# andimarafioti/faster-qwen3-tts

Hardware: AMD Instinct MI355X
Metric: real-time factor (audio s / wall s), Qwen3-TTS-12Hz-0.6B voice-clone streaming chunk_size=8; p50 TTFA in ttfa_ms_p50 (higher is better)
Workload: dtype bf16

## Files before the change

### faster-qwen3-tts_amd/csrc/fq3_api.hip

```cpp
#define FQ3_SKINNY_EXTERN
#include "fq3_ctx.h"
#include "sampler.cuh"
#include "sampler_wave.cuh"
#include "skinny_gemm.cuh"
#include "state_kernels.cuh"

#include <cstdio>
#include <cstdlib>
#include <cstring>
#include <map>
#include <string>
#include <type_traits>
#include <vector>

using namespace fq3;

static thread_local std::string g_err;
static int fail(int code, const std::string& m) { g_err = m; return code; }
int fq3_fail_(int code, const std::string& m) { return fail(code, m); }
#define HIPCHK(x) do { hipError_t e_ = (x); if (e_ != hipSuccess) return fail(FQ3_EHIP, std::string(#x) + ": " + hipGetErrorString(e_)); } while (0)

extern "C" const char* fq3_last_error(void) { return g_err.c_str(); }
extern "C" void fq3_set_error_(const char* msg) { g_err = msg ? msg : ""; }
extern "C" int fq3_abi_version(void) { return FQ3_ABI_VERSION; }
// ... 196 lines not shown
    if ((r = dmalloc(c, &c->past_hidden, (size_t)t.hidden * c->esz))) return r;
    if ((r = dmalloc(c, &c->ph_hold, (size_t)t.hidden * c->esz))) return r;
    if ((r = dmalloc(c, &c->pred_in, (size_t)2 * t.hidden * c->esz))) return r;
    if ((r = dmalloc(c, &c->pred_next, (size_t)t.hidden * c->esz))) return r;
    if ((r = dmalloc(c, &c->pred_x, (size_t)p.hidden * c->esz))) return r;
    if ((r = dmalloc(c, &c->plogits, (size_t)(G - 1) * p.vocab * c->esz))) return r;
    const int maxkv = std::max(t.n_kv_heads, p.n_kv_heads);
    c->part_stride = (size_t)maxkv * kMaxWorkers * 4 * kPartStride;
    if ((r = dmalloc(c, (void**)&c->part, 2 * c->part_stride * sizeof(float)))) return r;
    if ((r = dmalloc(c, (void**)&c->rope_now, 2 * 64 * sizeof(float)))) return r;
    if ((r = dmalloc(c, (void**)&c->seen_api, kMaxVocab))) return r;
    if ((r = dmalloc(c, (void**)&c->st, sizeof(DecodeState)))) return r;
    if ((r = dmalloc(c, (void**)&c->seen, kMaxVocab))) return r;
    if ((r = dmalloc(c, (void**)&c->codes, (size_t)(frames + 1) * G * sizeof(int)))) return r;
    if ((r = dmalloc(c, (void**)&c->ids64, (size_t)64 * sizeof(int64_t)))) return r;
    if ((r = dmalloc(c, (void**)&c->d_pemb, (size_t)64 * sizeof(void*)))) return r;
    HIPCHK(hipStreamCreateWithFlags(&c->cap_stream, hipStreamNonBlocking));
    return FQ3_OK;
}

extern "C" int fq3_set_option(fq3_ctx* c, const char* key, int value) {
    if (!c || !key) return fail(FQ3_EINVAL, "null argument");
    const std::string k(key);
    if (k == "weight_nt") c->opt_nt = value;
    else if (k == "pred_m2") c->opt_m2 = value;
    else if (k == "pred_attn") c->opt_pred_attn = value;
    else if (k == "rows_per_wave_max") c->opt_rmax = value;
    else if (k == "prefill_mode") c->prefill_mode = value;
    else if (k == "flash_prefill") c->opt_flash_prefill = value;
    else if (k == "flash_small") c->opt_flash_small = value;
    else if (k == "cont_pack") c->opt_cont_pack = value;
    else if (k == "swiglu_tile") c->opt_swiglu_tile = value;
    else if (k == "packed_weights") c->opt_packed = value;
    else if (k == "skinny_gemm") c->opt_no_skinny = !value;
    else return fail(FQ3_EINVAL, "unknown option: " + k);
    fq3_graph_reset(c);
    return FQ3_OK;
}

extern "C" int fq3_graph_reset(fq3_ctx* c) {
    if (!c) return fail(FQ3_EINVAL, "null ctx");
    if (c->exec) { (void)hipGraphExecDestroy(c->exec); c->exec = nullptr; }
    if (c->graph) { (void)hipGraphDestroy(c->graph); c->graph = nullptr; }
    return FQ3_OK;
}

namespace {
struct PackedEntry { void* p; int refs; int N, K; };
std::mutex g_packed_mu;
std::map<std::pair<const void*, int>, PackedEntry> g_packed;
}
const void* fq3_packed_find_(const void* W, int kind) {
    std::lock_guard<std::mutex> lk(g_packed_mu);
    auto it = g_packed.find({W, kind});
    return it == g_packed.end() ? nullptr : it->second.p;
}
int fq3_packed_acquire_(const void* W, int N, int K, int kind) {
    if (!W || !skinny_pack_ok(N, K) || (kind == 1 && (N / 2) % 8) || (kind == 2 && N % 512)) return FQ3_EUNSUPPORTED;
    std::lock_guard<std::mutex> lk(g_packed_mu);
    auto it = g_packed.find({W, kind});
    if (it != g_packed.end()) {
        if (it->second.N != N || it->second.K != K) return fail(FQ3_EINVAL, "a matrix is bound with two different shapes");
        ++it->second.refs;
        return FQ3_OK;
    }
    void* p = nullptr;
    if (hipMalloc(&p, (size_t)N * K * 2) != hipSuccess) { (void)hipGetLastError(); return fail(FQ3_ENOMEM, "no device memory for the fragment-major weight copy"); }
    skinny_pack(reinterpret_cast<const bf16_t*>(W), reinterpret_cast<bf16_t*>(p), N, K, kind == 1 ? N / 2 : (kind == 2 ? -(N / 2) : 0), nullptr);
    if (hipStreamSynchronize(nullptr) != hipSuccess) { (void)hipFree(p); return fail(FQ3_EHIP, "packing a weight matrix failed"); }
    g_packed[{W, kind}] = PackedEntry{p, 1, N, K};
    return FQ3_OK;
}
void fq3_packed_release_(const void* W, int kind) {
    std::lock_guard<std::mutex> lk(g_packed_mu);
    auto it = g_packed.find({W, kind});
    if (it == g_packed.end()) return;
    if (--it->second.refs <= 0) { (void)hipFree(it->second.p); g_packed.erase(it); }
}
static void packed_release_all(fq3_ctx* c) {
    for (auto& r : c->packed_refs) fq3_packed_release_(r.first, r.second);
    c->packed_refs.clear();
}
static int packed_acquire_all(fq3_ctx* c) {
    if (c->cfg.dtype != FQ3_BF16) return FQ3_OK;
    auto take = [&](const void* W, int N, int K, int kind) -> int {
        const int r = fq3_packed_acquire_(W, N, K, kind);
        if (r == FQ3_OK) c->packed_refs.emplace_back(W, kind);
        return r == FQ3_EUNSUPPORTED ? FQ3_OK : r;
    };
    auto stack = [&](const std::vector<fq3_layer_weights>& L, const fq3_stack_dims& d) -> int {
        const int qd = d.n_heads * kHeadDim, kvd = d.n_kv_heads * kHeadDim;
        for (const fq3_layer_weights& l : L) {
            if (int r = take(l.qkv, qd + 2 * kvd, d.hidden, 0)) return r;
            if (int r = take(l.o, d.hidden, qd, 0)) return r;
            if (int r = take(l.gate_up, 2 * d.inter, d.hidden, 1)) return r;
            if (int r = take(l.gate_up, 2 * d.inter, d.hidden, 0)) return r;
            if (int r = take(l.down, d.hidden, d.inter, 0)) return r;
        }
        return FQ3_OK;
    };
    if (int r = stack(c->tl, c->cfg.talker)) return r;
    if (int r = stack(c->pl, c->cfg.predictor)) return r;
    for (const fq3_layer_weights& l : c->tl) if (int r = take(l.gate_up, 2 * c->cfg.talker.inter, c->cfg.talker.hidden, 2)) return r;
    if (int r = take(c->wt.codec_head, c->cfg.talker.vocab, c->cfg.talker.hidden, 0)) return r;
    for (const void* h : c->lmh) if (int r = take(h, c->cfg.predictor.vocab, c->cfg.predictor.hidden, 0)) return r;
    return FQ3_OK;
}

extern "C" int fq3_ctx_destroy(fq3_ctx* c) {
    if (!c) return FQ3_OK;
    (void)hipDeviceSynchronize();
    fq3_graph_reset(c);
    packed_release_all(c);
    if (c->cap_stream) (void)hipStreamDestroy(c->cap_stream);
    if (fq3_kv_pool* p = c->tk.pool) {
        (void)fq3_kv_release(c, 0);
        bool last;
        { std::lock_guard<std::mutex> lk(p->mu); last = --p->users == 0; }
        if (p->is_private && last) pool_free_(p);
    }
    for (void* p : c->allocs) (void)hipFree(p);
    delete c;
    return FQ3_OK;
}

extern "C" int fq3_bind_weights(fq3_ctx* c, const fq3_weight_table* w) {
    if (!c || !w) return fail(FQ3_EINVAL, "null argument");
    const int G = c->cfg.num_code_groups;
    if (!w->talker_layers || !w->predictor_layers || !w->codec_embedding || !w->codec_head || !w->talker_final_norm ||
        !w->predictor_final_norm || !w->predictor_embeddings || !w->lm_heads || !w->talker_cos || !w->talker_sin ||
        !w->pred_cos || !w->pred_sin)
        return fail(FQ3_EINVAL, "weight table has null entries");
    if (c->cfg.has_projection && !w->proj_w) return fail(FQ3_EINVAL, "has_projection set but proj_w is null");
    if (w->talker_rope_len < c->cfg.max_seq_len || w->pred_rope_len < G + 1)
        return fail(FQ3_EINVAL, "rope tables shorter than the caches");
    c->wt = *w;
    c->tl.assign(w->talker_layers, w->talker_layers + c->cfg.talker.n_layers);
    c->pl.assign(w->predictor_layers, w->predictor_layers + c->cfg.predictor.n_layers);
    c->pemb.assign(w->predictor_embeddings, w->predictor_embeddings + (G - 1));
    c->lmh.assign(w->lm_heads, w->lm_heads + (G - 1));
    for (auto& l : c->tl) if (!l.qkv || !l.o || !l.gate_up || !l.down || !l.input_norm || !l.post_norm || !l.q_norm || !l.k_norm)
        return fail(FQ3_EINVAL, "talker layer has null weights");
    for (auto& l : c->pl) if (!l.qkv || !l.o || !l.gate_up || !l.down || !l.input_norm || !l.post_norm || !l.q_norm || !l.k_norm)
        return fail(FQ3_EINVAL, "predictor layer has null weights");
    HIPCHK(hipMemcpy(c->d_pemb, c->pemb.data(), (G - 1) * sizeof(void*), hipMemcpyHostToDevice));
    (void)hipDeviceSynchronize();
    packed_release_all(c);
    if (int r = packed_acquire_all(c)) { packed_release_all(c); return r; }
    c->bound = true;
    fq3_graph_reset(c);
    return FQ3_OK;
}

template <typename T, int NCH, int PRO, int EPI, bool NT, int M = 1>
static void launch_gemv_n(const GemvArgs& a, int rmax, hipStream_t s) {
    const int R = gemv_rows_per_wave<NCH, EPI>(a.N, rmax);
    const int grid = gemv_grid(a.N, R);
    const size_t shm = gemv_lds_bytes<PRO, M>(a.K);
    if constexpr (MaxRows<NCH, EPI>::v >= 2) {
        if (R == 2) { gemv_launch<T, NCH, PRO, EPI, NT, M, 2>(a, grid, shm, s); return; }
    }
    gemv_launch<T, NCH, PRO, EPI, NT, M, 1>(a, grid, shm, s);
}
template <typename T, int PRO, int EPI>
static int launch_gemv2_t(const GemvArgs& a, int rmax, hipStream_t s) {
    constexpr int most = gemv_most_chunks(PRO, 2);
    const int n = gemv_chunks(a.K, most);
    if (!n) return fail(FQ3_EUNSUPPORTED, PRO == PRO_NORM ? "code predictor hidden size above 2048" : "code predictor GEMV inner dimension above 3072");
    with_value<1, 2, 4, 6>(n, [&](auto nch) {
        if constexpr (decltype(nch)::value <= most) launch_gemv_n<T, decltype(nch)::value, PRO, EPI, false, 2>(a, rmax, s);
    });
    return 0;
}
template <int PRO, int EPI>
static int launch_gemv2(const fq3_ctx* c, const GemvArgs& a, hipStream_t s) {
    return c->cfg.dtype == FQ3_BF16 ? launch_gemv2_t<bf16_t, PRO, EPI>(a, c->opt_rmax, s) : launch_gemv2_t<float, PRO, EPI>(a, c->opt_rmax, s);
}
template <typename T, int PRO, int EPI, bool NT>
static int launch_gemv_t(const GemvArgs& a, int rmax, hipStream_t s) {
    constexpr int most = gemv_most_chunks(PRO, 1);
    const int n = gemv_chunks(a.K, most);
    if (!n) return fail(FQ3_EUNSUPPORTED, PRO == PRO_NORM ? "hidden size above 2048" : "GEMV inner dimension above 6144");
    with_value<1, 2, 4, 6, 12>(n, [&](auto nch) {
        if constexpr (decltype(nch)::value <= most) launch_gemv_n<T, decltype(nch)::value, PRO, EPI, NT>(a, rmax, s);
    });
    return 0;
}
template <int PRO, int EPI>
static int launch_gemv(const fq3_ctx* c, const GemvArgs& a, bool nt, hipStream_t s) {
    const int rmax = c->opt_rmax;
    if (c->cfg.dtype == FQ3_BF16)
        return nt ? launch_gemv_t<bf16_t, PRO, EPI, true>(a, rmax, s) : launch_gemv_t<bf16_t, PRO, EPI, false>(a, rmax, s);
    return nt ? launch_gemv_t<float, PRO, EPI, true>(a, rmax, s) : launch_gemv_t<float, PRO, EPI, false>(a, rmax, s);
}

template <typename T, bool PAGED>
static void launch_attn_p(const AttnArgs& a, int rep, int workers, hipStream_t s) {
    with_value<1, 2, 4>(rep, [&](auto r) {
        attn_decode_launch<T, decltype(r)::value, PAGED>(a, workers, s);
    });
}
template <typename T>
static void launch_attn_t(const AttnArgs& a, int rep, int workers, hipStream_t s) {
    if (a.table) launch_attn_p<T, true>(a, rep, workers, s); else launch_attn_p<T, false>(a, rep, workers, s);
}

struct StepSrc { const void* x0; const int* pos_ptr; int pos_imm; bool kv_only_tail = false; };

static int run_stack(fq3_ctx* c, bool talker, const StepSrc& src, hipStream_t s) {
    const fq3_stack_dims& d = talker ? c->cfg.talker : c->cfg.predictor;
    const std::vector<fq3_layer_weights>& L = talker ? c->tl : c->pl;
    StackBufs& kv = talker ? c->tk : c->pk;
    const int rep = d.n_heads / d.n_kv_heads;
    const int q_dim = d.n_heads * kHeadDim, kv_dim = d.n_kv_heads * kHeadDim;
    const bool nt = c->opt_nt == 2 || (c->opt_nt == 1 && talker);
    const float *cos_row, *sin_row;
    if (src.pos_ptr) { cos_row = c->rope_now; sin_row = c->rope_now + 64; }
    else {
        const int rl = talker ? c->wt.talker_rope_len : c->wt.pred_rope_len;
        int rp = src.pos_imm + (talker ? c->rope_delta : 0);
        rp = rp < 0 ? 0 : (rp >= rl ? rl - 1 : rp);
        cos_row = (talker ? c->wt.talker_cos : c->wt.pred_cos) + (size_t)rp * 64;
        sin_row = (talker ? c->wt.talker_sin : c->wt.pred_sin) + (size_t)rp * 64;
    }
    for (int i = 0; i < d.n_layers; ++i) {
        const fq3_layer_weights& w = L[i];
        const void* xin = i == 0 ? src.x0 : c->h;
        GemvArgs g{};
        g.eps = d.rms_eps;
        g.W = w.qkv; g.N = q_dim + 2 * kv_dim; g.K = d.hidden; g.x = xin;
        g.norm_w = w.input_norm; g.y = c->qkv;
        if (int r = launch_gemv<PRO_NORM, EPI_STORE>(c, g, nt, s)) return r;
        const bool tail_skip = src.kv_only_tail && i == d.n_layers - 1;
        GemvArgs o{};
        o.W = w.o; o.N = d.hidden; o.K = q_dim; o.y = c->h; o.res = xin; o.rep = rep;
        AttnArgs a{};
        a.qkv = c->qkv; a.q_norm_w = w.q_norm; a.k_norm_w = w.k_norm; a.eps = d.rms_eps;
        a.cos_row = cos_row; a.sin_row = sin_row;
        a.kcache = kv.k[i]; a.vcache = kv.v[i]; a.max_seq = kv.max_seq;
        a.table = kv.d_table; a.blk_stride = kv.pool ? (int)kv.pool->blk_elems : 0;
        a.pos_ptr = src.pos_ptr; a.pos_imm = src.pos_imm;
        a.done_ptr = src.pos_ptr ? &c->st->done : nullptr;
        a.n_pad = talker ? c->n_pad : 0;
        a.n_kv = d.n_kv_heads; a.part = c->part;
        a.scale = 1.0f / sqrtf((float)kHeadDim);
        a.rep = rep; a.out = c->attn_out;
        const bool pred_attn = c->opt_pred_attn && !talker && !src.pos_ptr && src.pos_imm <= 16;
        if (pred_attn) {
            if (c->cfg.dtype == FQ3_BF16) attn_pred_launch<bf16_t>(a, d.n_heads, s);
            else attn_pred_launch<float>(a, d.n_heads, s);
            if (tail_skip) break;
            o.x = c->attn_out;
            if (int r = launch_gemv<PRO_PLAIN, EPI_RESIDUAL>(c, o, nt, s)) return r;
        } else {
            if (c->cfg.dtype == FQ3_BF16) launch_attn_t<bf16_t>(a, rep, kv.workers, s);
            else launch_attn_t<float>(a, rep, kv.workers, s);
            if (tail_skip) break;
            o.part = c->part; o.n_part = kv.workers;
            if (int r = launch_gemv<PRO_COMBINE, EPI_RESIDUAL>(c, o, nt, s)) return r;
        }
        GemvArgs m{};
        m.eps = d.rms_eps; m.W = w.gate_up; m.N = d.inter; m.K = d.hidden; m.x = c->h;
        m.norm_w = w.post_norm; m.y = c->act; m.up_off = d.inter;
        if (int r = launch_gemv<PRO_NORM, EPI_SWIGLU>(c, m, nt, s)) return r;
        GemvArgs dn{};
// ... 364 lines not shown
                g_err = m;
                return r;
            }
    }
    if (walk) {
        for (int q = 0; q < n; ++q)
            if (int r = fq3_prefill_continue(ctxs[q], embeds[q], start[q], cnt[q], out_logits ? out_logits[q] : nullptr, out_hidden[q], stream)) return r;
        return FQ3_OK;
    }
    for (int q = 0; q < n; ++q)
        if (int r = fq3_set_generation_state(ctxs[q], 0, 0)) return r;
    if (int r = fq3_prefill_continue_batch_mfma_(ctxs, n, embeds, start, cnt, out_logits, out_hidden, s)) return r;
    LAUNCH_CHECK();
    return FQ3_OK;
}

int fq3_codec_head_launch_(fq3_ctx* c, const void* hidden, void* out_logits, hipStream_t s) {
    GemvArgs g{};
    g.W = c->wt.codec_head; g.N = c->cfg.talker.vocab; g.K = c->cfg.talker.hidden; g.x = hidden; g.y = out_logits;
    return launch_gemv<PRO_PLAIN, EPI_STORE>(c, g, true, s);
}

extern "C" int fq3_set_prefill_mode(fq3_ctx* c, int mode) { return fq3_set_option(c, "prefill_mode", mode); }

__global__ void build_seen_kernel(const int64_t* history, int n, unsigned char* seen, int V) {
    for (int i = threadIdx.x; i < V; i += blockDim.x) seen[i] = 0;
    __syncthreads();
    for (int i = threadIdx.x; i < n; i += blockDim.x) { const int id = (int)history[i]; if (id >= 0 && id < V) seen[id] = 1; }
}

template <typename T>
static void launch_sample_pred(const DecodeState* st, const T* lg, int V, int cb, const SampleCfg& cfg, const T* nz,
                               int* codes, int G, int64_t* out64, const T* next_emb, T* next_in, int H, bool wave,
                               const TeacherForcing* tf, hipStream_t s) {
    if (wave) dispatch_nc(V, [&](auto nc) {
        constexpr int NC = decltype(nc)::value;
        sample_pred_wave_launch<T, NC>(st, lg, V, cb, cfg, nz, codes, G, out64, next_emb, next_in, H, tf, s);
    });
    else hipLaunchKernelGGL((sample_pred_kernel<T>), dim3(1), dim3(256), 0, s, st, lg, V, cb, cfg, nz, codes, G, out64,
                            next_emb, next_in, H, tf);
}
template <typename T>
static void launch_sample_talker(DecodeState* st, const T* lg, int V, const unsigned char* seen, int G, bool wave,
                                 const TeacherForcing* tf, hipStream_t s) {
    if (wave) dispatch_nc(V, [&](auto nc) {
        constexpr int NC = decltype(nc)::value;
        sample_talker_wave_launch<T, NC>(st, lg, V, seen, G, tf, s);
    });
    else hipLaunchKernelGGL((sample_talker_kernel<T>), dim3(1), dim3(256), 0, s, st, lg, V, seen, G, tf);
}
template <typename T>
static void launch_sample_api(fq3_ctx* c, const T* lg, int V, const SampleCfg& cfg, const int64_t* history, int n_hist,
                              const T* noise, int64_t* out, hipStream_t s) {
    if (cfg.top_p >= 1.0f) {
        const unsigned char* seen = nullptr;
        if (n_hist > 0) {
            hipLaunchKernelGGL(build_seen_kernel, dim3(1), dim3(256), 0, s, history, n_hist, c->seen_api, V);
            seen = c->seen_api;
        }
        dispatch_nc(V, [&](auto nc) {
            constexpr int NC = decltype(nc)::value;
            hipLaunchKernelGGL((sample_api_wave_kernel<T, NC>), dim3(1), dim3(256), 0, s, lg, V, cfg, seen, noise, out);
        });
    } else {
        hipLaunchKernelGGL((sample_api_kernel<T>), dim3(1), dim3(256), 0, s, lg, V, cfg, history, n_hist, noise, out);
    }
}

static SampleCfg to_cfg(const fq3_sampling& s) {
    SampleCfg c{};
// ... 20 lines not shown
    LAUNCH_CHECK();
    return FQ3_OK;
}

template <typename T>
__global__ __launch_bounds__(256) void rep_penalty_kernel(T* logits, int V, const unsigned char* seen, float penalty) {
    for (int i = threadIdx.x; i < V; i += 256) {
        if (!seen[i]) continue;
        const float v = DT<T>::ld(logits + i);
        DT<T>::st(logits + i, v > 0.f ? v / penalty : v * penalty);
    }
}
extern "C" int fq3_apply_repetition_penalty(fq3_ctx* c, void* logits, int V, const int64_t* history, int n_hist,
                                            float penalty, void* stream) {
    if (!c || !logits) return fail(FQ3_EINVAL, "null argument");
    if (V <= 0 || V > kMaxVocab) return fail(FQ3_EUNSUPPORTED, "vocab must be at most 4096");
    if (penalty == 1.0f || n_hist <= 0 || !history) return FQ3_OK;
    hipStream_t s = (hipStream_t)stream;
    hipLaunchKernelGGL(build_seen_kernel, dim3(1), dim3(256), 0, s, history, n_hist, c->seen_api, V);
    if (c->cfg.dtype == FQ3_BF16) hipLaunchKernelGGL((rep_penalty_kernel<bf16_t>), dim3(1), dim3(256), 0, s, (bf16_t*)logits, V, c->seen_api, penalty);
    else hipLaunchKernelGGL((rep_penalty_kernel<float>), dim3(1), dim3(256), 0, s, (float*)logits, V, c->seen_api, penalty);
    LAUNCH_CHECK();
    return FQ3_OK;
}

extern "C" int fq3_set_predictor_sampling(fq3_ctx* c, const fq3_sampling* s) {
    if (!c || !s) return fail(FQ3_EINVAL, "null argument");
    if (s->do_sample && !(s->temperature > 0.f)) return fail(FQ3_EINVAL, "temperature must be > 0");
    if ((s->top_p >= 1.0f) != (c->pred_sampling.top_p >= 1.0f)) fq3_graph_reset(c);
    c->pred_sampling = *s;
    return FQ3_OK;
}

template <typename T>
static int predictor_passes_t(fq3_ctx* c, const DecodeState* st_dev, const void* pred_input, const void* noise_imm,
                              int64_t* out64, void* out_logits, hipStream_t s) {
    const fq3_stack_dims &p = c->cfg.predictor, &t = c->cfg.talker;
    const int G = c->cfg.num_code_groups, Vp = p.vocab, Ht = t.hidden;
    SampleCfg scfg = to_cfg(c->pred_sampling);
    for (int pass = 0; pass < G; ++pass) {
        const void* hsrc = c->h;
        if (pass == 0 && c->opt_m2) {
            const T* xa = (const T*)pred_input;
            const T* xb = (const T*)pred_input + Ht;
            if (c->cfg.has_projection) {
                GemvArgs g{};
                g.W = c->wt.proj_w; g.bias = c->wt.proj_b; g.N = p.hidden; g.K = Ht; g.x = xa; g.x2 = xb; g.y = c->pred_x; g.y2 = c->pred_x2;
                if (int r = launch_gemv2<PRO_PLAIN, EPI_STORE>(c, g, s)) return r;
                xa = (const T*)c->pred_x; xb = (const T*)c->pred_x2;
            }
            if (int r = run_predictor_pair(c, xa, xb, s)) return r;
            pass = 1;
            hsrc = c->h2;
        } else {
        const T* x_talker = pass < 2 ? (const T*)pred_input + (size_t)pass * Ht : (const T*)c->pred_next;
        const void* x0 = x_talker;
        if (c->cfg.has_projection) {
            GemvArgs g{};
            g.W = c->wt.proj_w; g.bias = c->wt.proj_b; g.N = p.hidden; g.K = Ht; g.x = x_talker; g.y = c->pred_x;
            if (int r = launch_gemv<PRO_PLAIN, EPI_STORE>(c, g, false, s)) return r;
            x0 = c->pred_x;
        }
        StepSrc src{x0, nullptr, pass};
        src.kv_only_tail = pass == 0;
        if (int r = run_stack(c, false, src, s)) return r;
        }
        if (pass == 0) continue;
        const int cb = pass - 1;
        T* lg = out_logits ? (T*)out_logits + (size_t)cb * Vp : (T*)c->plogits + (size_t)cb * Vp;
        GemvArgs hgm{};
        hgm.eps = p.rms_eps; hgm.W = c->lmh[cb]; hgm.N = Vp; hgm.K = p.hidden; hgm.x = hsrc;
        hgm.norm_w = c->wt.predictor_final_norm; hgm.y = lg;
        if (int r = launch_gemv<PRO_NORM, EPI_STORE>(c, hgm, false, s)) return r;
        const T* nz = noise_imm ? (const T*)noise_imm + (size_t)cb * Vp : nullptr;
        const T* next_emb = cb + 1 < G - 1 ? (const T*)c->pemb[cb] : nullptr;
        launch_sample_pred<T>(st_dev, (const T*)lg, Vp, cb, scfg, nz, st_dev ? c->codes : nullptr, G, out64, next_emb,
                              (T*)c->pred_next, Ht, c->pred_sampling.top_p >= 1.0f, st_dev ? c->tf : nullptr, s);
    }
    return 0;
}

extern "C" int fq3_predictor_loop(fq3_ctx* c, const void* pred_input, const void* noise, int64_t* out_ids,
                                  void* out_logits, void* stream) {
    NEED_BOUND(c);
    if (!pred_input || !out_ids) return fail(FQ3_EINVAL, "null argument");
    if (c->pred_sampling.do_sample && !noise) return fail(FQ3_EINVAL, "predictor sampling enabled but no noise given");
    hipStream_t s = (hipStream_t)stream;
    int r = c->cfg.dtype == FQ3_BF16 ? predictor_passes_t<bf16_t>(c, nullptr, pred_input, noise, out_ids, out_logits, s)
                                     : predictor_passes_t<float>(c, nullptr, pred_input, noise, out_ids, out_logits, s);
    if (r) return r;
    LAUNCH_CHECK();
    return FQ3_OK;
}

extern "C" int fq3_decode_begin(fq3_ctx* c, const fq3_decode_params* p, void* stream) {
    NEED_BOUND(c);
    if (!p || !p->past_hidden || !p->tts_pad_embed) return fail(FQ3_EINVAL, "null argument");
    if (p->trailing_len > 0 && !p->trailing_text) return fail(FQ3_EINVAL, "trailing_text");
    if (p->talker.do_sample && (!p->talker_noise || p->noise_frames <= 0)) return fail(FQ3_EINVAL, "talker sampling needs a noise ring");
    if (c->pred_sampling.do_sample && (!p->pred_noise || p->noise_frames <= 0)) return fail(FQ3_EINVAL, "predictor sampling needs a noise ring");
    if (p->talker.do_sample && !(p->talker.temperature > 0.f)) return fail(FQ3_EINVAL, "temperature must be > 0");
    if (p->max_new_tokens > c->cfg.max_frames) return fail(FQ3_EINVAL, "max_new_tokens exceeds the context's max_frames");
    if (p->prefill_len <= 0 || p->prefill_len > c->cfg.max_seq_len) return fail(FQ3_EINVAL, "prefill_len");
    if (p->first_token < 0 || p->first_token >= c->cfg.talker.vocab) return fail(FQ3_EINVAL, "first_token outside the codec vocabulary");
    if (p->gen_step < 0 || p->min_new_tokens < 0 || p->max_new_tokens < 0) return fail(FQ3_EINVAL, "negative counters");
    const bool wave = p->talker.top_p >= 1.0f;
    if (wave != c->talker_wave) { fq3_graph_reset(c); c->talker_wave = wave; }
    hipStream_t s = (hipStream_t)stream;
    if (int r = fq3_kv_ensure_(c, p->prefill_len + p->max_new_tokens + 1, s)) return r;
    DecodeState h{};
    h.token = p->first_token; h.frame = 0; h.pos = p->prefill_len; h.gen_step = p->gen_step; h.done = 0; h.text_open = 0;
    h.min_new = p->min_new_tokens; h.max_new = p->max_new_tokens; h.trailing_len = p->trailing_len;
    h.noise_frames = p->noise_frames > 0 ? p->noise_frames : 1;
    h.eos_id = c->cfg.codec_eos_token_id; h.max_seq = c->cfg.max_seq_len;
    h.n_pad = c->n_pad; h.rope_delta = c->rope_delta;
    h.sup_lo = c->cfg.talker.vocab - 1024 > 0 ? c->cfg.talker.vocab - 1024 : 0; h.sup_hi = c->cfg.talker.vocab;
    h.t_temperature = p->talker.temperature; h.t_top_k = p->talker.top_k; h.t_top_p = p->talker.top_p;
    h.t_do_sample = p->talker.do_sample; h.t_rep_penalty = p->talker.repetition_penalty;
    h.p_temperature = c->pred_sampling.temperature; h.p_top_k = c->pred_sampling.top_k; h.p_top_p = c->pred_sampling.top_p;
    h.p_do_sample = c->pred_sampling.do_sample;
// ... 27 lines not shown

template <typename T>
static int enqueue_frame_t(fq3_ctx* c, hipStream_t s) {
    const fq3_stack_dims& t = c->cfg.talker;
    const int G = c->cfg.num_code_groups, H = t.hidden;
    DecodeState* st = c->st;
    frame_begin_launch<T>(st, (const T*)c->wt.codec_embedding, (const T*)c->past_hidden, (T*)c->ph_hold, (T*)c->pred_in, c->codes, c->seen,
                          H, G, s);
    if (int r = predictor_passes_t<T>(c, st, c->pred_in, nullptr, nullptr, nullptr, s)) return r;
    EmbTables tabs{};
    tabs.t[0] = c->wt.codec_embedding;
    for (int i = 1; i < G; ++i) tabs.t[i] = c->pemb[i - 1];
    if (G != 16) return fail(FQ3_EUNSUPPORTED, "the fused loop is built for 16 code groups");
    embed_sum_launch<T, 16>(st, tabs, c->codes, (T*)c->xin, H, c->wt.talker_cos, c->wt.talker_sin, c->wt.talker_rope_len, c->rope_delta,
                            c->rope_now, s);
    StepSrc src{c->xin, &st->pos, 0};
    if (int r = run_stack(c, true, src, s)) return r;
    GemvArgs g{};
    g.eps = t.rms_eps; g.W = c->wt.codec_head; g.N = t.vocab; g.K = H; g.x = c->h;
    g.norm_w = c->wt.talker_final_norm; g.y = c->logits; g.xn_out = c->past_hidden;
    if (int r = launch_gemv<PRO_NORM, EPI_STORE>(c, g, true, s)) return r;
    launch_sample_talker<T>(st, (const T*)c->logits, t.vocab, c->seen, G, c->talker_wave, c->tf, s);
    return 0;
}
static int enqueue_frame(fq3_ctx* c, hipStream_t s) {
    return c->cfg.dtype == FQ3_BF16 ? enqueue_frame_t<bf16_t>(c, s) : enqueue_frame_t<float>(c, s);
}

extern "C" int fq3_graph_capture(fq3_ctx* c, void* stream) {
    NEED_BOUND(c);
    if (c->exec) return FQ3_OK;
    (void)stream;
    hipStream_t cs = c->cap_stream;
    HIPCHK(hipStreamBeginCapture(cs, hipStreamCaptureModeRelaxed));
    int r = enqueue_frame(c, cs);
    hipGraph_t g = nullptr;
    hipError_t e = hipStreamEndCapture(cs, &g);
    if (r) { if (g) (void)hipGraphDestroy(g); return r; }
    if (e != hipSuccess) return fail(FQ3_EHIP, std::string("hipStreamEndCapture: ") + hipGetErrorString(e));
    c->graph = g;
    HIPCHK(hipGraphInstantiate(&c->exec, c->graph, nullptr, nullptr, 0));
    return FQ3_OK;
}

extern "C" int fq3_decode_frames(fq3_ctx* c, int n_frames, void* stream) {
    NEED_BOUND(c);
    hipStream_t s = (hipStream_t)stream;
    for (int i = 0; i < n_frames; ++i) {
        if (c->exec) { HIPCHK(hipGraphLaunch(c->exec, s)); }
        else if (int r = enqueue_frame(c, s)) return r;
    }
    LAUNCH_CHECK();
    return FQ3_OK;
}

extern "C" int fq3_decode_poll(fq3_ctx* c, int* n_frames_total, int* done, void* stream) {
    if (!c) return fail(FQ3_EINVAL, "null ctx");
    hipStream_t s = (hipStream_t)stream;
    DecodeState h;
    HIPCHK(hipMemcpyAsync(&h, c->st, sizeof h, hipMemcpyDeviceToHost, s));
    HIPCHK(hipStreamSynchronize(s));
    if (n_frames_total) *n_frames_total = h.frame;
    if (done) *done = h.done == 2 ? 2 : (h.done || h.token == h.eos_id);
    return FQ3_OK;
}

extern "C" int fq3_decode_codes(fq3_ctx* c, int from, int count, int64_t* out, void* stream) {
    if (!c || !out) return fail(FQ3_EINVAL, "null argument");
    if (from < 0 || count < 0 || from + count > c->cfg.max_frames) return fail(FQ3_EINVAL, "range");
    const int G = c->cfg.num_code_groups, n = count * G;
    if (n == 0) return FQ3_OK;
    hipLaunchKernelGGL(codes_to_i64_kernel, dim3((n + 255) / 256), dim3(256), 0, (hipStream_t)stream,
                       c->codes + (size_t)from * G, out, n);
    LAUNCH_CHECK();
    return FQ3_OK;
}
```

### faster-qwen3-tts_amd/csrc/fq3_ctx.h

```cpp
#pragma once
#include "../../include/fq3hip.h"
#include "decode_kernels.cuh"
#include <hip/hip_runtime.h>
#include <mutex>
#include <string>
#include <utility>
#include <vector>

struct fq3_kv_pool {
    int dtype = 0, esz = 2, n_layers = 0, n_kv = 0, n_blocks = 0;
    size_t blk_elems = 0;
    std::vector<void*> k, v;
    std::vector<int> free_list;
    std::mutex mu;
    int in_use_high = 0;
    int users = 0;
    bool is_private = false;
};

struct StackBufs {
    std::vector<void*> k, v;
    int max_seq = 0, workers = 1;
    fq3_kv_pool* pool = nullptr;
    int* d_table = nullptr;
// ... 4 lines not shown
struct fq3_ctx {
    fq3_config cfg{};
    int esz = 2;
    std::vector<fq3_layer_weights> tl, pl;
    fq3_weight_table wt{};
    std::vector<const void*> pemb, lmh;
    const void** d_pemb = nullptr;
    bool bound = false;
    StackBufs tk, pk;
    void *h = nullptr, *xin = nullptr, *qkv = nullptr, *act = nullptr, *logits = nullptr, *past_hidden = nullptr;
    void *pred_in = nullptr, *pred_x = nullptr, *pred_next = nullptr, *plogits = nullptr, *tmp_hidden = nullptr;
    void *attn_out = nullptr, *attn_out2 = nullptr;
    void *h2 = nullptr, *qkv2 = nullptr, *act2 = nullptr, *pred_x2 = nullptr;
    size_t part_stride = 0;
    float* part = nullptr;
    float* rope_now = nullptr;
    unsigned char* seen_api = nullptr;
    fq3::DecodeState* st = nullptr;
    fq3::TeacherForcing* tf = nullptr;
    unsigned char* seen = nullptr;
    int* codes = nullptr;
    int64_t* ids64 = nullptr;
    int n_pad = 0, rope_delta = 0;
    int opt_nt = 1;
    int opt_m2 = 1;
    int opt_pred_attn = 1;
    int opt_rmax = 2;
    int opt_flash_prefill = 1;
    int opt_flash_small = 1;
    int opt_cont_pack = 1;
    int opt_swiglu_tile = 1;
    int opt_packed = 1;
    std::vector<std::pair<const void*, int>> packed_refs;
    int opt_no_skinny = 0;
    int prefill_mode = 0;
    bool talker_wave = true;
    fq3_sampling pred_sampling{0.9f, 50, 1.0f, 1, 1.0f};
    hipGraph_t graph = nullptr;
    hipGraphExec_t exec = nullptr;
    hipStream_t cap_stream = nullptr;
    std::vector<void*> allocs;
    fq3_prompt_weights pw{};
    bool pw_bound = false;
    void *pw_x = nullptr, *pw_h = nullptr;
    int pw_cap = 0;
    void* ph_hold = nullptr;
    void *tt_tab = nullptr, *tt_x = nullptr, *tt_h = nullptr;
    int tt_alloc = 0;
    int tt_cap = 0, tt_rows = 0;
    bool tt_open = false, tt_session = false;
    bool armed = false;
    const void* begin_trailing = nullptr; int begin_trailing_len = 0;
    void *pf_x = nullptr, *pf_xn = nullptr, *pf_qkv = nullptr, *pf_att = nullptr, *pf_gu = nullptr, *pf_act = nullptr, *pf_ws = nullptr;
};


const void* fq3_packed_find_(const void* W, int kind);
int fq3_packed_acquire_(const void* W, int N, int K, int kind);
void fq3_packed_release_(const void* W, int kind);

int fq3_fail_(int code, const std::string& m);
int fq3_kv_ensure_(fq3_ctx* c, int n_pos, hipStream_t s);
int fq3_prefill_reserve_(fq3_ctx* c);
int fq3_prefill_mfma_(fq3_ctx* c, const void* embeds, int L, int n_pad, void* out_logits, void* out_hidden, hipStream_t s);
int fq3_prefill_continue_mfma_(fq3_ctx* c, const void* embeds, int start, int n, void* out_logits, void* out_hidden, hipStream_t s);
int fq3_prefill_continue_batch_mfma_(fq3_ctx* const* cs, int n, const void* const* embeds, const int* start, const int* cnt,
// ... 7 lines not shown
```

### faster-qwen3-tts_amd/csrc/sampler_wave.cuh

```cuda
#pragma once
#include "sampler.cuh"
#include <type_traits>

namespace fq3 {

__device__ __forceinline__ ArgMax wave_argmax(ArgMax a) {
    ArgMax r;
    r.v = wave_max(a.v);
    r.i = wave_min_i32(a.v == r.v ? a.i : 0x7fffffff);
    return r;
}

struct BlkSmem { int cnt[2][4]; float f[4]; float av[4]; int ai[4]; };

__device__ __forceinline__ float blk_max4(float v, BlkSmem& sm) {
    v = wave_max(v);
    __syncthreads();
    if ((threadIdx.x & 63) == 0) sm.f[threadIdx.x >> 6] = v;
    __syncthreads();
    return fmaxf(fmaxf(sm.f[0], sm.f[1]), fmaxf(sm.f[2], sm.f[3]));
}
__device__ __forceinline__ float blk_sum4(float v, BlkSmem& sm) {
    v = wave_sum(v);
    __syncthreads();
// ... 125 lines not shown
        if (off < V) ldraw<false>(xraw[j], logits + off); else zero(xraw[j]);
    }
}

template <typename T, int NC>
__global__ __launch_bounds__(256) void sample_api_wave_kernel(const T* logits, int V, SampleCfg c, const unsigned char* seen,
                                                             const T* noise, int64_t* out) {
    __shared__ BlkSmem sm;
    Raw8<T> xraw[NC];
    issue_logits<T, NC>(xraw, logits, V);
    const int tok = sample_wave_core<T, NC>(xraw, V, c, seen, noise, sm);
    if (threadIdx.x == 0) out[0] = tok;
}

template <typename T, int NC>
__device__ __forceinline__ int sample_nucleus_from_regs(Raw8<T> (&xraw)[NC], int V, const SampleCfg& c, const unsigned char* seen,
                                                        const T* noise, SampleSmem& big) {
#pragma unroll
    for (int j = 0; j < NC; ++j) {
        float f[8];
        unpack(xraw[j], f);
#pragma unroll
        for (int i = 0; i < 8; ++i) {
            const int id = j * 2048 + threadIdx.x * 8 + i;
            if (id < V) big.vals[id] = f[i];
        }
    }
    __syncthreads();
    const int tok = sample_core<T>(big, V, c, seen, noise);
    __syncthreads();
    return tok;
}

template <typename T, int NC, bool NUCLEUS = false>
__device__ __forceinline__ void sample_pred_wave_body(const DecodeState* st, const T* logits, int V, int cb,
                                                      const SampleCfg& c_imm, const T* noise_imm, int* codes, int G,
                                                      int64_t* out64, const T* next_emb, T* next_in, int H, const TeacherForcing* tf = nullptr) {
    __shared__ BlkSmem sm;
    Raw8<T> xraw[NC];
    issue_logits<T, NC>(xraw, logits, V);
    SampleCfg c = c_imm;
    const T* noise = noise_imm;
    int frame = 0;
    if (st) {
        if (st->done) return;
        c.temperature = st->p_temperature; c.top_k = st->p_top_k; c.top_p = st->p_top_p; c.do_sample = st->p_do_sample;
        frame = st->frame;
        if (st->pred_noise)
            noise = gptr(reinterpret_cast<const T*>(st->pred_noise)) + ((size_t)(frame % st->noise_frames) * (G - 1) + cb) * V;
    }
    int tok;
    if constexpr (NUCLEUS) {
        __shared__ SampleSmem big;
        if (c.do_sample && c.top_p < 1.0f) tok = sample_nucleus_from_regs<T, NC>(xraw, V, c, nullptr, noise, big);
        else tok = sample_wave_core<T, NC>(xraw, V, c, nullptr, noise, sm);
    } else {
        tok = sample_wave_core<T, NC>(xraw, V, c, nullptr, noise, sm);
    }
    if (st) tok = forced_or(tf, frame * G + 1 + cb, tok);
    if (threadIdx.x == 0) {
        if (codes) codes[(size_t)frame * G + 1 + cb] = tok;
        if (out64) out64[cb] = tok;
    }
    if (next_emb) {
        const T* src = next_emb + (size_t)tok * H;
        for (int e = threadIdx.x * 8; e < H; e += 256 * 8) {
            Raw8<T> r; ldraw<false>(r, src + e);
            if (sizeof(T) == 2) *reinterpret_cast<u32x4*>(reinterpret_cast<char*>(next_in) + (size_t)e * 2) = *reinterpret_cast<u32x4*>(&r);
            else { float f[8]; unpack(r, f);
#pragma unroll
                   for (int i = 0; i < 8; ++i) DT<T>::st(next_in + e + i, f[i]); }
        }
    }
}

constexpr int kSamplePredLeadDwords = 14;
template <typename T, int NC>
__global__ __launch_bounds__(256) void sample_pred_wave_kernel(const DecodeState* st, const T* logits, const T* noise_imm, int* codes,
                                                              int64_t* out64, const T* next_emb, int V, int cb, int G, int H,
                                                              T* next_in, const TeacherForcing* tf, SampleCfg c_imm) {
    sample_pred_wave_body<T, NC>(st, logits, V, cb, c_imm, noise_imm, codes, G, out64, next_emb, next_in, H, tf);
}
template <typename T, int NC>
inline void sample_pred_wave_launch(const DecodeState* st, const T* logits, int V, int cb, const SampleCfg& c_imm, const T* noise_imm,
                                    int* codes, int G, int64_t* out64, const T* next_emb, T* next_in, int H, const TeacherForcing* tf,
                                    hipStream_t s) {
    hipLaunchKernelGGL((sample_pred_wave_kernel<T, NC>), dim3(1), dim3(256), 0, s, st, logits, noise_imm, codes, out64, next_emb, V, cb, G, H,
                       next_in, tf, c_imm);
}

template <typename T, int NC, bool NUCLEUS = false>
__device__ __forceinline__ void sample_talker_wave_body(DecodeState* st, const T* logits, int V, const unsigned char* seen, int G,
                                                        const TeacherForcing* tf = nullptr) {
    __shared__ BlkSmem sm;
    Raw8<T> xraw[NC];
    issue_logits<T, NC>(xraw, logits, V);
    if (st->done) return;
    SampleCfg c;
    c.temperature = st->t_temperature; c.top_k = st->t_top_k; c.top_p = st->t_top_p; c.do_sample = st->t_do_sample;
    c.rep_penalty = st->t_rep_penalty;
    c.sup_lo = st->sup_lo; c.sup_hi = st->sup_hi; c.keep_id = st->eos_id;
    const int frame = st->frame;
    c.sup_extra = (frame + 1 < st->min_new) ? st->eos_id : -1;
    const T* noise = st->talker_noise
        ? gptr(reinterpret_cast<const T*>(st->talker_noise)) + (size_t)(frame % st->noise_frames) * V : nullptr;
    int tok;
    if constexpr (NUCLEUS) {
        __shared__ SampleSmem big;
        if (c.do_sample && c.top_p < 1.0f) tok = sample_nucleus_from_regs<T, NC>(xraw, V, c, seen, noise, big);
        else tok = sample_wave_core<T, NC>(xraw, V, c, seen, noise, sm);
    } else {
        tok = sample_wave_core<T, NC>(xraw, V, c, seen, noise, sm);
    }
    tok = forced_or(tf, (frame + 1) * G, tok);
    if (threadIdx.x == 0) { st->token = tok; st->frame = frame + 1; st->pos += 1; st->gen_step += 1; }
}
constexpr int kSampleTalkerLeadDwords = 10;
template <typename T, int NC>
__global__ __launch_bounds__(256) void sample_talker_wave_kernel(DecodeState* st, const T* logits, const unsigned char* seen,
                                                                const TeacherForcing* tf, int V, int G) {
    sample_talker_wave_body<T, NC>(st, logits, V, seen, G, tf);
// ... 9 lines not shown
```

Before: 39.11.

## Precompute predictor layer-0 QKV rows per codebook token and gather them in the sampler

Builds a one-time device table holding, for every codebook and predictor token, the projected embedding and the RMS-normed layer-0 QKV output. The table depends only on the weights, and both the projection and the per-row norm are exact functions of the token embedding. In predictor passes from 2 onward, the sampler kernel copies the matching rows straight into the qkv and pred_x buffers, so the projection GEMV and the first QKV GEMV are skipped. This removes two kernel launches and their weight reads per codebook pass. The cost is a large extra device allocation, a slow first-call fill, and a path that only applies when top_p is 1.

```diff
diff --git a/faster-qwen3-tts_amd/csrc/fq3_api.hip b/faster-qwen3-tts_amd/csrc/fq3_api.hip
--- a/faster-qwen3-tts_amd/csrc/fq3_api.hip
+++ b/faster-qwen3-tts_amd/csrc/fq3_api.hip
@@ -252,6 +252,7 @@
     else if (k == "cont_pack") c->opt_cont_pack = value;
     else if (k == "swiglu_tile") c->opt_swiglu_tile = value;
     else if (k == "packed_weights") c->opt_packed = value;
+    else if (k == "pred_qkv_table") c->opt_pred_tab = value;
     else if (k == "skinny_gemm") c->opt_no_skinny = !value;
     else return fail(FQ3_EINVAL, "unknown option: " + k);
     fq3_graph_reset(c);
@@ -297,6 +298,7 @@
     if (it == g_packed.end()) return;
     if (--it->second.refs <= 0) { (void)hipFree(it->second.p); g_packed.erase(it); }
 }
+static void pred_tab_release(fq3_ctx* c);
 static void packed_release_all(fq3_ctx* c) {
     for (auto& r : c->packed_refs) fq3_packed_release_(r.first, r.second);
     c->packed_refs.clear();
@@ -332,6 +334,7 @@
     (void)hipDeviceSynchronize();
     fq3_graph_reset(c);
     packed_release_all(c);
+    pred_tab_release(c);
     if (c->cap_stream) (void)hipStreamDestroy(c->cap_stream);
     if (fq3_kv_pool* p = c->tk.pool) {
         (void)fq3_kv_release(c, 0);
@@ -366,6 +369,7 @@
     HIPCHK(hipMemcpy(c->d_pemb, c->pemb.data(), (G - 1) * sizeof(void*), hipMemcpyHostToDevice));
     (void)hipDeviceSynchronize();
     packed_release_all(c);
+    pred_tab_release(c);
     if (int r = packed_acquire_all(c)) { packed_release_all(c); return r; }
     c->bound = true;
     fq3_graph_reset(c);
@@ -425,7 +429,7 @@
     if (a.table) launch_attn_p<T, true>(a, rep, workers, s); else launch_attn_p<T, false>(a, rep, workers, s);
 }
 
-struct StepSrc { const void* x0; const int* pos_ptr; int pos_imm; bool kv_only_tail = false; };
+struct StepSrc { const void* x0; const int* pos_ptr; int pos_imm; bool kv_only_tail = false; bool qkv_ready = false; };
 
 static int run_stack(fq3_ctx* c, bool talker, const StepSrc& src, hipStream_t s) {
     const fq3_stack_dims& d = talker ? c->cfg.talker : c->cfg.predictor;
@@ -450,7 +454,8 @@
         g.eps = d.rms_eps;
         g.W = w.qkv; g.N = q_dim + 2 * kv_dim; g.K = d.hidden; g.x = xin;
         g.norm_w = w.input_norm; g.y = c->qkv;
-        if (int r = launch_gemv<PRO_NORM, EPI_STORE>(c, g, nt, s)) return r;
+        if (!(i == 0 && src.qkv_ready))
+            if (int r = launch_gemv<PRO_NORM, EPI_STORE>(c, g, nt, s)) return r;
         const bool tail_skip = src.kv_only_tail && i == d.n_layers - 1;
         GemvArgs o{};
         o.W = w.o; o.N = d.hidden; o.K = q_dim; o.y = c->h; o.res = xin; o.rep = rep;
@@ -881,10 +886,10 @@
 template <typename T>
 static void launch_sample_pred(const DecodeState* st, const T* lg, int V, int cb, const SampleCfg& cfg, const T* nz,
                                int* codes, int G, int64_t* out64, const T* next_emb, T* next_in, int H, bool wave,
-                               const TeacherForcing* tf, hipStream_t s) {
+                               const TeacherForcing* tf, hipStream_t s, const PredRowTable<T>& tab = PredRowTable<T>{}) {
     if (wave) dispatch_nc(V, [&](auto nc) {
         constexpr int NC = decltype(nc)::value;
-        sample_pred_wave_launch<T, NC>(st, lg, V, cb, cfg, nz, codes, G, out64, next_emb, next_in, H, tf, s);
+        sample_pred_wave_launch<T, NC>(st, lg, V, cb, cfg, nz, codes, G, out64, next_emb, next_in, H, tf, s, tab);
     });
     else hipLaunchKernelGGL((sample_pred_kernel<T>), dim3(1), dim3(256), 0, s, st, lg, V, cb, cfg, nz, codes, G, out64,
                             next_emb, next_in, H, tf);
@@ -971,12 +976,92 @@
     return FQ3_OK;
 }
 
+namespace {
+struct PredTabEntry { void* qkv; void* x; int refs; };
+std::mutex g_pred_tab_mu;
+std::map<std::pair<const void*, const void*>, PredTabEntry> g_pred_tab;
+}
+static int pred_qkv_width(const fq3_ctx* c) { return (c->cfg.predictor.n_heads + 2 * c->cfg.predictor.n_kv_heads) * kHeadDim; }
+static bool pred_tab_fits(const fq3_ctx* c) {
+    const int Ht = c->cfg.talker.hidden, Hp = c->cfg.predictor.hidden, w = pred_qkv_width(c);
+    if (c->cfg.num_code_groups < 3 || c->cfg.predictor.vocab <= 0 || c->pl.empty()) return false;
+    if (Ht % 8 || Ht > 2048 || w % 8 || w > kPredRowTrips * 2048) return false;
+    if (c->cfg.has_projection ? (Hp % 8 || Hp > 2048) : Hp != Ht) return false;
+    return true;
+}
+static int pred_tab_fill(fq3_ctx* c, void* qkv, void* x) {
+    const fq3_stack_dims &p = c->cfg.predictor, &t = c->cfg.talker;
+    const int n_cb = c->cfg.num_code_groups - 2, Vp = p.vocab, w = pred_qkv_width(c);
+    const bool nt = c->opt_nt == 2;
+    hipStream_t s = nullptr;
+    for (int cb = 0; cb < n_cb; ++cb)
+        for (int tok = 0; tok < Vp; ++tok) {
+            const size_t row = (size_t)cb * Vp + tok;
+            const void* x0 = (const char*)c->pemb[cb] + (size_t)tok * t.hidden * c->esz;
+            if (c->cfg.has_projection) {
+                GemvArgs g{};
+                g.W = c->wt.proj_w; g.bias = c->wt.proj_b; g.N = p.hidden; g.K = t.hidden; g.x = x0; g.y = (char*)x + row * p.hidden * c->esz;
+                if (int r = launch_gemv<PRO_PLAIN, EPI_STORE>(c, g, false, s)) return r;
+                x0 = g.y;
+            }
+            GemvArgs g{};
+            g.eps = p.rms_eps; g.W = c->pl[0].qkv; g.N = w; g.K = p.hidden; g.x = x0; g.norm_w = c->pl[0].input_norm;
+            g.y = (char*)qkv + row * w * c->esz;
+            if (int r = launch_gemv<PRO_NORM, EPI_STORE>(c, g, nt, s)) return r;
+        }
+    if (hipGetLastError() != hipSuccess || hipStreamSynchronize(s) != hipSuccess) { (void)hipGetLastError(); return FQ3_EHIP; }
+    return FQ3_OK;
+}
+static void pred_tab_release(fq3_ctx* c) {
+    c->pred_tab_tried = false;
+    if (!c->pred_tab_qkv) return;
+    std::lock_guard<std::mutex> lk(g_pred_tab_mu);
+    auto it = g_pred_tab.find({c->pred_tab_key, c->pred_tab_key2});
+    if (it != g_pred_tab.end() && --it->second.refs <= 0) {
+        (void)hipFree(it->second.qkv);
+        if (it->second.x) (void)hipFree(it->second.x);
+        g_pred_tab.erase(it);
+    }
+    c->pred_tab_qkv = c->pred_tab_x = nullptr;
+}
+static void pred_tab_ensure(fq3_ctx* c, hipStream_t s) {
+    if (!c->opt_pred_tab || c->pred_tab_tried) return;
+    hipStreamCaptureStatus cap = hipStreamCaptureStatusNone;
+    if (hipStreamIsCapturing(s, &cap) != hipSuccess || cap != hipStreamCaptureStatusNone) { (void)hipGetLastError(); return; }
+    c->pred_tab_tried = true;
+    if (!pred_tab_fits(c)) return;
+    const std::pair<const void*, const void*> key{c->pl[0].qkv, c->pemb[0]};
+    std::lock_guard<std::mutex> lk(g_pred_tab_mu);
+    auto it = g_pred_tab.find(key);
+    if (it == g_pred_tab.end()) {
+        const size_t rows = (size_t)(c->cfg.num_code_groups - 2) * c->cfg.predictor.vocab;
+        void *qkv = nullptr, *x = nullptr;
+        (void)hipDeviceSynchronize();
+        bool ok = hipMalloc(&qkv, rows * pred_qkv_width(c) * c->esz) == hipSuccess;
+        if (ok && c->cfg.has_projection) ok = hipMalloc(&x, rows * c->cfg.predictor.hidden * c->esz) == hipSuccess;
+        if (ok) { const std::string m = g_err; ok = pred_tab_fill(c, qkv, x) == FQ3_OK; g_err = m; }
+        if (!ok) {
+            (void)hipGetLastError();
+            if (qkv) (void)hipFree(qkv);
+            if (x) (void)hipFree(x);
+            return;
+        }
+        it = g_pred_tab.emplace(key, PredTabEntry{qkv, x, 0}).first;
+    }
+    ++it->second.refs;
+    c->pred_tab_key = key.first; c->pred_tab_key2 = key.second;
+    c->pred_tab_qkv = it->second.qkv; c->pred_tab_x = it->second.x;
+}
+
 template <typename T>
 static int predictor_passes_t(fq3_ctx* c, const DecodeState* st_dev, const void* pred_input, const void* noise_imm,
                               int64_t* out64, void* out_logits, hipStream_t s) {
     const fq3_stack_dims &p = c->cfg.predictor, &t = c->cfg.talker;
     const int G = c->cfg.num_code_groups, Vp = p.vocab, Ht = t.hidden;
     SampleCfg scfg = to_cfg(c->pred_sampling);
+    const bool wave = c->pred_sampling.top_p >= 1.0f;
+    const bool use_tab = c->opt_pred_tab && c->pred_tab_qkv && wave;
+    const int qkv_w = pred_qkv_width(c);
     for (int pass = 0; pass < G; ++pass) {
         const void* hsrc = c->h;
         if (pass == 0 && c->opt_m2) {
@@ -994,14 +1079,17 @@
         } else {
         const T* x_talker = pass < 2 ? (const T*)pred_input + (size_t)pass * Ht : (const T*)c->pred_next;
         const void* x0 = x_talker;
+        const bool from_tab = use_tab && pass >= 2;
         if (c->cfg.has_projection) {
             GemvArgs g{};
             g.W = c->wt.proj_w; g.bias = c->wt.proj_b; g.N = p.hidden; g.K = Ht; g.x = x_talker; g.y = c->pred_x;
-            if (int r = launch_gemv<PRO_PLAIN, EPI_STORE>(c, g, false, s)) return r;
+            if (!from_tab)
+                if (int r = launch_gemv<PRO_PLAIN, EPI_STORE>(c, g, false, s)) return r;
             x0 = c->pred_x;
         }
         StepSrc src{x0, nullptr, pass};
         src.kv_only_tail = pass == 0;
+        src.qkv_ready = from_tab;
         if (int r = run_stack(c, false, src, s)) return r;
         }
         if (pass == 0) continue;
@@ -1013,8 +1101,13 @@
         if (int r = launch_gemv<PRO_NORM, EPI_STORE>(c, hgm, false, s)) return r;
         const T* nz = noise_imm ? (const T*)noise_imm + (size_t)cb * Vp : nullptr;
         const T* next_emb = cb + 1 < G - 1 ? (const T*)c->pemb[cb] : nullptr;
+        PredRowTable<T> tab{};
+        if (use_tab && next_emb) {
+            tab.qkv = (const T*)c->pred_tab_qkv + (size_t)cb * Vp * qkv_w; tab.qkv_out = (T*)c->qkv; tab.qkv_w = qkv_w;
+            if (c->pred_tab_x) { tab.x = (const T*)c->pred_tab_x + (size_t)cb * Vp * p.hidden; tab.x_out = (T*)c->pred_x; tab.x_w = p.hidden; }
+        }
         launch_sample_pred<T>(st_dev, (const T*)lg, Vp, cb, scfg, nz, st_dev ? c->codes : nullptr, G, out64, next_emb,
-                              (T*)c->pred_next, Ht, c->pred_sampling.top_p >= 1.0f, st_dev ? c->tf : nullptr, s);
+                              (T*)c->pred_next, Ht, wave, st_dev ? c->tf : nullptr, s, tab);
     }
     return 0;
 }
@@ -1025,6 +1118,7 @@
     if (!pred_input || !out_ids) return fail(FQ3_EINVAL, "null argument");
     if (c->pred_sampling.do_sample && !noise) return fail(FQ3_EINVAL, "predictor sampling enabled but no noise given");
     hipStream_t s = (hipStream_t)stream;
+    pred_tab_ensure(c, s);
     int r = c->cfg.dtype == FQ3_BF16 ? predictor_passes_t<bf16_t>(c, nullptr, pred_input, noise, out_ids, out_logits, s)
                                      : predictor_passes_t<float>(c, nullptr, pred_input, noise, out_ids, out_logits, s);
     if (r) return r;
@@ -1118,6 +1212,7 @@
     if (c->exec) return FQ3_OK;
     (void)stream;
     hipStream_t cs = c->cap_stream;
+    pred_tab_ensure(c, cs);
     HIPCHK(hipStreamBeginCapture(cs, hipStreamCaptureModeRelaxed));
     int r = enqueue_frame(c, cs);
     hipGraph_t g = nullptr;
@@ -1132,6 +1227,7 @@
 extern "C" int fq3_decode_frames(fq3_ctx* c, int n_frames, void* stream) {
     NEED_BOUND(c);
     hipStream_t s = (hipStream_t)stream;
+    if (!c->exec && n_frames > 0) pred_tab_ensure(c, s);
     for (int i = 0; i < n_frames; ++i) {
         if (c->exec) { HIPCHK(hipGraphLaunch(c->exec, s)); }
         else if (int r = enqueue_frame(c, s)) return r;
diff --git a/faster-qwen3-tts_amd/csrc/fq3_ctx.h b/faster-qwen3-tts_amd/csrc/fq3_ctx.h
--- a/faster-qwen3-tts_amd/csrc/fq3_ctx.h
+++ b/faster-qwen3-tts_amd/csrc/fq3_ctx.h
@@ -60,6 +60,10 @@
     int opt_swiglu_tile = 1;
     int opt_packed = 1;
     std::vector<std::pair<const void*, int>> packed_refs;
+    int opt_pred_tab = 1;
+    const void *pred_tab_qkv = nullptr, *pred_tab_x = nullptr;
+    const void *pred_tab_key = nullptr, *pred_tab_key2 = nullptr;
+    bool pred_tab_tried = false;
     int opt_no_skinny = 0;
     int prefill_mode = 0;
     bool talker_wave = true;
diff --git a/faster-qwen3-tts_amd/csrc/sampler_wave.cuh b/faster-qwen3-tts_amd/csrc/sampler_wave.cuh
--- a/faster-qwen3-tts_amd/csrc/sampler_wave.cuh
+++ b/faster-qwen3-tts_amd/csrc/sampler_wave.cuh
@@ -181,10 +181,23 @@
     return tok;
 }
 
+constexpr int kPredRowTrips = 4;
+template <typename T>
+struct PredRowTable {
+    const T* qkv = nullptr; T* qkv_out = nullptr; int qkv_w = 0;
+    const T* x = nullptr; T* x_out = nullptr; int x_w = 0;
+};
+template <typename T>
+__device__ __forceinline__ void st_raw8(T* dst, const Raw8<T>& r) {
+    if constexpr (sizeof(T) == 2) *reinterpret_cast<u32x4*>(dst) = r.v;
+    else { reinterpret_cast<f32x4*>(dst)[0] = r.a; reinterpret_cast<f32x4*>(dst)[1] = r.b; }
+}
+
 template <typename T, int NC, bool NUCLEUS = false>
 __device__ __forceinline__ void sample_pred_wave_body(const DecodeState* st, const T* logits, int V, int cb,
                                                       const SampleCfg& c_imm, const T* noise_imm, int* codes, int G,
-                                                      int64_t* out64, const T* next_emb, T* next_in, int H, const TeacherForcing* tf = nullptr) {
+                                                      int64_t* out64, const T* next_emb, T* next_in, int H, const TeacherForcing* tf = nullptr,
+                                                      const PredRowTable<T>& tab = PredRowTable<T>{}) {
     __shared__ BlkSmem sm;
     Raw8<T> xraw[NC];
     issue_logits<T, NC>(xraw, logits, V);
@@ -211,7 +224,21 @@
         if (codes) codes[(size_t)frame * G + 1 + cb] = tok;
         if (out64) out64[cb] = tok;
     }
-    if (next_emb) {
+    if (next_emb && tab.qkv) {
+        const int e = threadIdx.x * 8;
+        const T* qsrc = tab.qkv + (size_t)tok * tab.qkv_w;
+        Raw8<T> re, rx, rq[kPredRowTrips];
+        if (e < H) ldraw<false>(re, next_emb + (size_t)tok * H + e);
+#pragma unroll
+        for (int j = 0; j < kPredRowTrips; ++j)
+            if (j * 2048 + e < tab.qkv_w) ldraw<false>(rq[j], qsrc + j * 2048 + e);
+        if (tab.x && e < tab.x_w) ldraw<false>(rx, tab.x + (size_t)tok * tab.x_w + e);
+        if (e < H) st_raw8(next_in + e, re);
+#pragma unroll
+        for (int j = 0; j < kPredRowTrips; ++j)
+            if (j * 2048 + e < tab.qkv_w) st_raw8(tab.qkv_out + j * 2048 + e, rq[j]);
+        if (tab.x && e < tab.x_w) st_raw8(tab.x_out + e, rx);
+    } else if (next_emb) {
         const T* src = next_emb + (size_t)tok * H;
         for (int e = threadIdx.x * 8; e < H; e += 256 * 8) {
             Raw8<T> r; ldraw<false>(r, src + e);
@@ -227,15 +254,15 @@
 template <typename T, int NC>
 __global__ __launch_bounds__(256) void sample_pred_wave_kernel(const DecodeState* st, const T* logits, const T* noise_imm, int* codes,
                                                               int64_t* out64, const T* next_emb, int V, int cb, int G, int H,
-                                                              T* next_in, const TeacherForcing* tf, SampleCfg c_imm) {
-    sample_pred_wave_body<T, NC>(st, logits, V, cb, c_imm, noise_imm, codes, G, out64, next_emb, next_in, H, tf);
+                                                              T* next_in, const TeacherForcing* tf, SampleCfg c_imm, PredRowTable<T> tab) {
+    sample_pred_wave_body<T, NC>(st, logits, V, cb, c_imm, noise_imm, codes, G, out64, next_emb, next_in, H, tf, tab);
 }
 template <typename T, int NC>
 inline void sample_pred_wave_launch(const DecodeState* st, const T* logits, int V, int cb, const SampleCfg& c_imm, const T* noise_imm,
                                     int* codes, int G, int64_t* out64, const T* next_emb, T* next_in, int H, const TeacherForcing* tf,
-                                    hipStream_t s) {
+                                    hipStream_t s, const PredRowTable<T>& tab = PredRowTable<T>{}) {
     hipLaunchKernelGGL((sample_pred_wave_kernel<T, NC>), dim3(1), dim3(256), 0, s, st, logits, noise_imm, codes, out64, next_emb, V, cb, G, H,
-                       next_in, tf, c_imm);
+                       next_in, tf, c_imm, tab);
 }
 
 template <typename T, int NC, bool NUCLEUS = false>
```

Measured after the change: 39.22 (median of 3 runs). Within noise of the previous version (+0.3%).
